# lxd99/TPNet

Measured on AMD Instinct MI355X. Metric: temporal edges/sec (proj-update + pairwise readout), higher is better.
Workload: dtype f32; 1 GPU; C2: Wikipedia-shape d=128 B=1000, L=3, synthetic S(8227,1000,E,span) stream of 2399000 edges, decoder-level unit (2 readouts + update per edge); batch=1000, dim=128, num_layer=3, nodes=9228, parallelism=single GPU

## Files before the change

tpnet_amd/csrc/plan.hip:

```cpp
#include "tpnet_common.h"

#include <cstdlib>
#include <cstring>
#include <rocprim/block/block_radix_sort.hpp>
#include <rocprim/device/device_radix_sort.hpp>
#include <rocprim/device/device_segmented_radix_sort.hpp>
#include <rocprim/iterator/counting_iterator.hpp>
#include <rocprim/iterator/transform_iterator.hpp>

#ifdef TPNET_STAMPS
#define PSTAMP(slot)                                                                          \
    do {                                                                                      \
        if (dbg && blockIdx.x == 0 && threadIdx.x == 0) {                                     \
            dbg[(slot) * 2 + 0] = __builtin_amdgcn_s_memtime();                               \
            dbg[(slot) * 2 + 1] = __builtin_amdgcn_s_memrealtime();                           \
        }                                                                                     \
    } while (0)
#else
#define PSTAMP(slot) do { } while (0)
#endif

namespace tpnet {

static constexpr uint32_t HEAVY_THRESHOLD = 8u;
// ... 900 lines not shown
    if (max_edges < 1) max_edges = 1;
    if (batch < 1) batch = 1;
    return plan_bytes(max_edges, batch) + wplan_extra_bytes(max_edges, batch, N, d, L, 2);
}

int wplan_carve(void* ws, size_t ws_bytes, int64_t Ec, int64_t batch, int64_t N, int d, int L, int K, WPlan* out, float* shared_log,
                bool shard) {
    if (K < 1 || K > WIN_MAX_BATCHES || (!shard && K > wplan_window_batches(batch, d, L))) return TPNET_ERR_BAD_ARG;
    if (Ec > wplan_max_chunk_edges(batch, d, L)) return TPNET_ERR_BAD_ARG;
    int rc = plan_carve(ws, ws_bytes, Ec, batch, &out->base);
    if (rc) return rc;
    const size_t base_bytes = plan_bytes(Ec, batch);
    if (base_bytes + wplan_extra_bytes(Ec, batch, N, d, L, K) - (shared_log ? wplan_log_bytes(Ec, d, L) : 0) > ws_bytes)
        return TPNET_ERR_WORKSPACE;
    char* p = reinterpret_cast<char*>(align_up(reinterpret_cast<size_t>(ws), 256)) + align_up(base_bytes, 256);
    auto take = [&](size_t bytes) -> void* {
        void* r = p;
        p += align_up(bytes, 256);
        return r;
    };
    const size_t nc = 2 * (size_t)Ec;
    const int64_t Ew = (int64_t)K * batch;
    const size_t nw = (size_t)((Ec + batch - 1) / batch);
    out->s_ref = (uint32_t*)take(nc * 4);
    out->s_g = (float*)take(nc * 4);
    out->s_dec = (float*)take(nc * 4);
    out->s_bc = (uint16_t*)take(nc * 2);
    out->wdesc = (WinDesc*)take(nw * sizeof(WinDesc));
    (void)take(256);
    out->e_ref = (uint32_t*)take(3 * (size_t)Ec * 4);
    out->e_g = (float*)take(3 * (size_t)Ec * 4);
    out->log = shared_log ? shared_log : (float*)take(nc * (size_t)L * (size_t)d * 4);
    out->node_lo = (uint32_t*)take((size_t)N * 4);
    out->node_hi = (uint32_t*)take((size_t)N * 4);
    out->inv = (uint32_t*)take(nc * 4);
    out->rhead = (uint32_t*)take(nc * 4);
    out->wmask = (unsigned long long*)take((size_t)N * 8);
    out->wcls = (uint32_t*)take((2 * WIN_MAX_WINDOWS * 8 + WIN_MAX_WINDOWS) * 4);
    out->wzero_bytes = (size_t)(p - reinterpret_cast<char*>(out->wmask));
    out->wtab = take(wplan3_table_bytes(Ec, batch));
    out->wblk = (uint32_t*)take(wplan3_blk_bytes(Ec, batch));
    {
        const size_t db = wplan_dense_bytes(Ec, batch, N, d, L);
        out->dense = db ? take(db) : nullptr;
    }
    out->heavy_thr = wplan_heavy_threshold(K, batch, d);
    out->chains = reinterpret_cast<Chain*>(out->base.light);
    out->chains_sparse = reinterpret_cast<Chain*>(out->base.heavy);
    out->lk_in = reinterpret_cast<uint32_t*>(out->base.keys_in);
    out->lk_out = out->lk_in + nc;
    out->lv_in = out->base.vals_in;
    out->lv_out = out->base.vals_out;
    out->K = K;
    out->Ew = Ew;
    if (p > reinterpret_cast<char*>(ws) + ws_bytes) return TPNET_ERR_WORKSPACE;
    return TPNET_OK;
}

template <typename K>
__global__ void k_make_keys_w(K* __restrict__ keys, uint32_t* __restrict__ vals, const int64_t* __restrict__ src,
                              const int64_t* __restrict__ dst, int64_t Ec, int64_t B, int64_t N, int batch_bits, DescArgs da) {
    if (blockIdx.x >= da.kblocks) {
        for (int64_t b = (int64_t)(blockIdx.x - da.kblocks) * blockDim.x + threadIdx.x; b < da.nb;
             b += (int64_t)(gridDim.x - da.kblocks) * blockDim.x)
            batch_desc(b, da.desc, da.t, Ec, B, da.nb, da.now_time, da.t_prev, da.lambda, da.L);
        return;
    }
    const int64_t nc = 2 * Ec;
    for (int64_t j = (int64_t)blockIdx.x * blockDim.x + threadIdx.x; j < nc; j += (int64_t)da.kblocks * blockDim.x) {
        int64_t b, e;
        int side;
// ... 103 lines not shown
                           const NodeMeta* __restrict__ meta, uint32_t* err) {
    const int64_t nc = 2 * Ec;
    const int KW = p.K;
    const K bmask = ((K)1 << batch_bits) - 1;
    const BatchDesc* __restrict__ desc = p.base.desc;
    for (int64_t jb = (int64_t)bx * blockDim.x; jb < nc; jb += (int64_t)nbx * blockDim.x) {
        const int64_t j = jb + threadIdx.x;
        const bool active = j < nc;
        bool chain_head = false, last_run = false;
        int64_t w = 0;
        if (active) lv[j] = (uint32_t)j;
        Chain ch;
        ch.j0 = 0; ch.cnt = 0; ch.target = 0; ch.prev_ref = WREF_TABLE; ch.g_first = 1.0f; ch.pad0 = 0; ch.pad1 = 0; ch.pad2 = 0;
        if (active) {
            const K key = keys[j];
            const uint32_t val = p.base.vals_out[j];
            const int64_t b = (int64_t)(key & bmask);
            const int64_t node = (int64_t)(key >> batch_bits);
            w = b / KW;
            const double Tb = desc[b].t_last;
            int32_t partner;
            float wgt;
            contribution(p.base, src, dst, t, Ec, B, N, lambda, val, partner, wgt, err);
            p.base.s_partner[j] = partner;
            p.base.s_coef[j] = wgt;
            p.s_bc[j] = (uint16_t)b;
            p.base.s_target[j] = (int32_t)node;

            const bool has_prev = j > 0, has_next = j < nc - 1;
            const K kp = has_prev ? keys[j - 1] : key, kn = has_next ? keys[j + 1] : key;
            const bool run_head = !has_prev || kp != key;
            const bool run_tail = !has_next || kn != key;
            const bool same_node_prev = has_prev && (kp >> batch_bits) == (key >> batch_bits);
            const bool same_node_next = has_next && (kn >> batch_bits) == (key >> batch_bits);
            chain_head = !same_node_prev || (int64_t)(kp & bmask) / KW != w;
            last_run = run_tail && !same_node_next;
            const int64_t h = p.rhead[j];
            const int64_t ri = j - h;
            uint32_t ref;
            float g;
            {
                int64_t cb, ce;
                int cside;
                decode((int64_t)val, B, Ec, cb, cside, ce);
                const int64_t e0b = cb * B;
                const int64_t neb = (Ec - e0b < B) ? (Ec - e0b) : B;
                const uint32_t sym = (uint32_t)(2 * e0b + (cside ? 0 : neb) + (ce - e0b));
                if (!version_before_own_run<K>(p, keys, batch_bits, (int64_t)partner, b, p.inv[sym], desc, meta, lambda, Tb, ref, g))
                    resolve_version(keys, nc, batch_bits, (int64_t)partner, b, desc, meta, lambda, Tb, ref, g, p.node_lo, p.node_hi);
            }
            uint32_t fl = 0;
            if (run_head) fl |= WREF_RUN_HEAD;
            if (run_tail) fl |= WREF_RUN_TAIL;
            if (ri % WIN_BLOCK == 0) fl |= WREF_BLK_HEAD;
            if (ri % WIN_BLOCK == WIN_BLOCK - 1 || run_tail) fl |= WREF_BLK_TAIL;
            if (last_run) fl |= WREF_LAST_RUN;
            p.s_ref[j] = ref | fl;
            p.s_g[j] = g;
            float dec = 1.0f;
            if (run_head && same_node_prev) dec = decay_f32(lambda, Tb - desc[(int64_t)(kp & bmask)].t_last);
            p.s_dec[j] = dec;

            if (chain_head) {
                const K bound = (K)(((uint64_t)node << batch_bits) | (uint64_t)((w + 1) * KW));
                const K node_end = (K)(((uint64_t)(node + 1)) << batch_bits);
                const K stop = ((uint64_t)((w + 1) * KW) > (uint64_t)bmask) ? node_end : bound;
                int64_t lo = j, hi, step = 1;
                for (;;) {
                    const int64_t nx = lo + step;
                    if (nx >= nc) { hi = nc; break; }
                    if (keys[nx] >= stop) { hi = nx; break; }
                    lo = nx;
                    step <<= 1;
                }
                while (hi - lo > 1) {
                    const int64_t mid = (lo + hi) >> 1;
                    if (keys[mid] < stop) lo = mid; else hi = mid;
                }
                ch.j0 = (uint32_t)j;
                ch.cnt = (uint32_t)(hi - j);
                ch.target = (int32_t)node;
                if (same_node_prev) {
                    ch.prev_ref = (uint32_t)(j - 1);
                    ch.g_first = 1.0f;
// ... 160 lines not shown
```

tpnet_amd/csrc/tpnet_common.h:

```cpp
#pragma once
#include <hip/hip_runtime.h>
#include <stdint.h>
#include <stdlib.h>
#include <initializer_list>
#include <new>
#include "../../include/tpnet_hip.h"
#include "tpnet_dev.h"
#include "event_set.hpp"

#ifdef TPNET_DEV
static inline int tpnet_dev_env_int(const char* name, int dflt) { const char* v = getenv(name); return v ? atoi(v) : dflt; }
#define TPNET_DEV_INT(NAME, DFLT) tpnet_dev_env_int("TPNET_DEV_" #NAME, (DFLT))
#define TPNET_DEV_STR(NAME) getenv("TPNET_DEV_" #NAME)
#else
#define TPNET_DEV_INT(NAME, DFLT) (DFLT)
#define TPNET_DEV_STR(NAME) ((const char*)nullptr)
#endif

namespace tpnet {

struct NodeMeta {
    uint32_t ver;
    uint32_t pad0;
    double tref[2];
// ... 197 lines not shown
    return 1 + (dl > 6 ? 6 : (dl < 0 ? 0 : dl));
}

struct WinDesc {
    uint32_t start;
    uint32_t n_heavy;
    uint32_t n_chains;
    uint32_t n_ext;
    uint32_t n_ext1;
    uint32_t n_med;
    uint32_t pad1, pad2;
};

struct Chain {
    uint32_t j0;
    uint32_t cnt;
    int32_t target;
    uint32_t prev_ref;
    float g_first;
    uint32_t pad0, pad1, pad2;
};
static_assert(sizeof(Chain) == 32, "Chain must be 32 bytes");

struct WPlan {
    Plan base;
    uint32_t* s_ref;
    float* s_g;
    float* s_dec;
    uint16_t* s_bc;
    WinDesc* wdesc;
    Chain* chains;
    Chain* chains_sparse;
    uint32_t* lk_in;
    uint32_t* lk_out;
    uint32_t* lv_in;
    uint32_t* lv_out;
    uint32_t* e_ref;
    float* e_g;
    float* log;
    uint32_t* node_lo;
    uint32_t* node_hi;
    uint32_t* inv;
    uint32_t* rhead;
    unsigned long long* wmask;
    uint32_t* wcls;
    void* wtab;
    size_t wzero_bytes;
    uint32_t* wblk;
    void* dense;
    uint32_t heavy_thr;
    int32_t K;
    int64_t Ew;
// ... 63 lines not shown
```

tpnet_amd/csrc/wplan3.hip:

```cpp
#include "wplan_common.hpp"

namespace tpnet {

size_t wplan3_table_bytes(int64_t Ec, int64_t batch) {
    const size_t nb = (size_t)((Ec + batch - 1) / batch);
    return wplan3_h2_bytes(Ec) + 256 + nb * wplan3_seg(batch) * sizeof(HEnt) + 256;
}
size_t wplan3_blk_bytes(int64_t Ec, int64_t batch) {
    const size_t nblk = (size_t)((Ec + batch - 1) / batch) * wplan3_bpb(batch);
    return 2 * nblk * 9 * sizeof(uint32_t) + 256;
}

template <int BS, int IPT>
__global__ __launch_bounds__(BS) void k_wsort(WTmp q, BatchDesc* __restrict__ desc, const int64_t* __restrict__ src_c,
                                              const int64_t* __restrict__ dst_c, const double* __restrict__ t_c, int64_t Ec,
                                              int32_t Bfull, int64_t N, int node_bits, double now_time,
                                              const double* __restrict__ t_prev, double lambda, int L, uint32_t* err, int KW) {
    __shared__ WSortShared<BS, IPT> sh;
    wsort_batch<BS, IPT, false>(sh, q, desc, src_c, dst_c, t_c, Ec, Bfull, N, node_bits, now_time, t_prev, lambda, L, err, KW,
                                (int64_t)blockIdx.x, nullptr);
}


__global__ __launch_bounds__(256) void k_wchains(WPlan p, WTmp q, int64_t Ec, int64_t Bfull, int64_t nb, uint32_t bpb) {
// ... 174 lines not shown
    o.fl = q.bflags[x];
    o.coef = q.bcoef[x];
    o.sb = q.bsb[x - o.ri];
    o.aux = q.rprevb[x - o.ri];
}

__device__ __forceinline__ void side_version(const WPlan& p, const WTmp& q, int64_t Bfull, int64_t w, const CEnt* ce,
                                             const NodeMeta* __restrict__ meta, OwnSide& o) {
    int64_t lb;
    chain_of(p, q, Bfull, ce, w, o.base, o.cnt, lb);
    if (o.sb) {
        o.ver.ref = o.base + o.sb - 1u;
        o.ver.t_src = p.base.desc[o.aux].t_last;
    } else {
        o.ver = version_before_window_m(p, q, Bfull, o.node, w, o.wm, meta);
    }
}

__device__ __forceinline__ void side_store(const WPlan& p, const WTmp& q, int64_t Bfull, int64_t Ec, int64_t e, int sd, int64_t b,
                                           int64_t w, int64_t e0b, double Tb, double Tnow, double lambda,
                                           const NodeMeta* __restrict__ meta, const uint32_t* cabs, int want_edges,
                                           const OwnSide me, const OwnSide other) {
    const uint32_t f = me.base + me.sb + me.ri;
    p.base.s_partner[f] = me.partner;
    p.base.s_coef[f] = me.coef;
    p.base.s_target[f] = (int32_t)me.node;
    p.s_bc[f] = (uint16_t)b;
    VRef pr = other.ver;
    if ((uint32_t)me.partner != other.node)
        pr = version_before_batch(p, q, Bfull, (int64_t)me.partner, b, meta);
    uint32_t out = (me.fl & WT_STRUCT_MASK) | pr.ref;
    float dec = 1.0f;
    if (me.fl & WREF_RUN_HEAD) {
        if (me.fl & WT_CHAIN_HEAD) {
            float g_first = 1.0f;
            if (me.ver.ref & WREF_TABLE) g_first = decay3_f32(lambda, Tb - me.ver.t_src);
            else dec = decay3_f32(lambda, Tb - me.ver.t_src);
            const int c = wchain_class(me.cnt, p.heavy_thr);
            const int64_t blk = b * q.bpb + (me.x - 2 * e0b) / 256;
            uint4* rec = reinterpret_cast<uint4*>(p.chains + (cabs[w * WCLS + c] + q.blkbase[blk * 9 + c] + me.aux));
            rec[0] = make_uint4(f, me.cnt, me.node, me.ver.ref);
            rec[1] = make_uint4(__float_as_uint(g_first), 0u, 0u, 0u);
        } else {
            dec = decay3_f32(lambda, Tb - me.ver.t_src);
        }
    }
    if ((me.fl & WT_WIN_LAST) && (w >= 63 || (me.wm >> (unsigned)(w + 1)) == 0ull)) out |= WREF_LAST_RUN;
    p.s_ref[f] = out;
    p.s_g[f] = decay3_f32(lambda, Tb - pr.t_src);
    p.s_dec[f] = dec;
    if (want_edges) {
        p.e_ref[(int64_t)sd * Ec + e] = me.ver.ref;
        p.e_g[(int64_t)sd * Ec + e] = decay3_f32(lambda, Tnow - me.ver.t_src);
    }
}

__global__ __launch_bounds__(256) void k_wrefs(WPlan p, WTmp q, const int64_t* __restrict__ neg, int64_t Ec, int64_t Bfull,
                                               int64_t nb, int64_t N, double lambda, const NodeMeta* __restrict__ meta,
                                               uint32_t fgrid, int want_edges) {
    const int KW = p.K;
    const BatchDesc* __restrict__ desc = p.base.desc;
    if (blockIdx.x >= fgrid) {
        for (int64_t e = (int64_t)(blockIdx.x - fgrid) * blockDim.x + threadIdx.x; e < Ec;
             e += (int64_t)(gridDim.x - fgrid) * blockDim.x) {
            int64_t node = neg[e];
            if ((uint64_t)node >= (uint64_t)N) node = 0;
            const int64_t b = e / Bfull;
            const VRef r = version_before_batch(p, q, Bfull, node, b, meta);
            p.e_ref[2 * Ec + e] = r.ref;
            p.e_g[2 * Ec + e] = decay3_f32(lambda, desc[b].now - r.t_src);
        }
        return;
    }
// ... 161 lines not shown
```

tpnet_amd/csrc/wplan_common.hpp:

```cpp
#pragma once
#include "tpnet_common.h"
#include "device_common.hpp"

#include <rocprim/block/block_radix_sort.hpp>

namespace tpnet {

static constexpr uint32_t WT_CHAIN_HEAD = 1u;
static constexpr uint32_t WT_WIN_LAST = 2u;
static constexpr uint32_t WT_STRUCT_MASK = WREF_RUN_HEAD | WREF_RUN_TAIL | WREF_BLK_HEAD | WREF_BLK_TAIL;
static constexpr int WCLS = 8;

struct HEnt {
    unsigned long long key;
    uint32_t a, b;
};
static_assert(sizeof(HEnt) == 16, "HEnt must be 16 bytes");
struct CEnt {
    unsigned long long key;
    unsigned long long mask;
    uint32_t xh;
    uint32_t cnt;
    uint32_t pad0, pad1;
};
static_assert(sizeof(CEnt) == 32, "CEnt must be 32 bytes");

#ifdef TPNET_STAMPS
#define WSTAMP(slot)                                                                          \
    do {                                                                                      \
// ... 24 lines not shown
    uint32_t n2;
    uint32_t* blkcnt;
    uint32_t* blkbase;
    uint32_t* boff;
    uint32_t* wtot;
    uint32_t bpb;
    unsigned long long* dbg;
};

static inline uint32_t wplan3_table_entries(size_t nc) { return (uint32_t)(2 * nc + 1021); }
static inline uint32_t wplan3_nc_block(int64_t batch) {
    const int64_t n2 = 2 * batch;
    return n2 <= 512 ? 512u : n2 <= 1024 ? 1024u : n2 <= 2048 ? 2048u : 4096u;
}
static inline uint32_t wplan3_seg(int64_t batch) { return wplan3_nc_block(batch) * 3; }
static inline size_t wplan3_h2_bytes(int64_t Ec) { return (size_t)wplan3_table_entries(2 * (size_t)Ec) * sizeof(CEnt); }
static inline uint32_t wplan3_bpb(int64_t batch) { return (uint32_t)((2 * batch + 255) / 256); }

static WTmp wtmp_of(const WPlan& p, size_t nc) {
    WTmp q;
    q.dbg = p.base.dbg;
    uint32_t* ki = reinterpret_cast<uint32_t*>(p.base.keys_in);
    uint32_t* ko = reinterpret_cast<uint32_t*>(p.base.keys_out);
    uint32_t* hv = reinterpret_cast<uint32_t*>(p.base.heavy);
    q.bkey = ki;
    q.bpart = reinterpret_cast<int32_t*>(ki + nc);
    q.bcoef = reinterpret_cast<float*>(ko);
    q.bval = p.base.vals_out;
    q.binv = p.inv;
    q.bsb = hv;
    q.bri = hv + nc;
    q.rprevb = hv + 2 * nc;
    q.bflags = hv + 3 * nc;
    const uint32_t cap = wplan3_table_entries(nc);
    q.h2 = reinterpret_cast<CEnt*>(p.wtab);
    q.h1 = reinterpret_cast<HEnt*>(reinterpret_cast<char*>(p.wtab) + (wplan3_h2_bytes((int64_t)(nc / 2)) + 255) / 256 * 256);
    q.hcap = cap;
    q.seg = 0;
    q.direct2 = 0;
    q.n2 = 0;
    q.boff = p.rhead;
    q.wtot = p.wcls;
    return q;
}

__device__ __forceinline__ float decay3_f32(double lambda, double dt) {
    const float x = (float)(-lambda * dt);
    return (x == 0.0f) ? 1.0f : expf(x);
}

__device__ __forceinline__ uint32_t hmix(unsigned long long k) {
    k ^= k >> 33;
    k *= 0xff51afd7ed558ccdULL;
    k ^= k >> 33;
    k *= 0xc4ceb9fe1a85ec53ULL;
    k ^= k >> 33;
// ... 293 lines not shown
```

tpnet_amd/csrc/wplan_dense.hip:

```cpp
#include "wplan_dense.hpp"

namespace tpnet {

static constexpr int64_t DENSE_SHARD_MAX_BATCH = 8192;
bool wplan_dense_eligible(int64_t N, int d, int L, int64_t batch) {
    static const int off = TPNET_DEV_INT(NO_PLAN_DENSE, 0);
    if (off || batch < 1 || batch > DENSE_SHARD_MAX_BATCH || N > (int64_t)DENSE_MAX_CHUNKS * 256) return false;
    return (int64_t)N * 12 <= batch * (int64_t)L * d * 4;
}

size_t wplan_dense_bytes(int64_t Ec, int64_t batch, int64_t N, int d, int L) {
    if (!wplan_dense_eligible(N, d, L, batch)) return 0;
    const size_t nb = (size_t)((Ec + batch - 1) / batch);
    const size_t Ns = (size_t)dense_ns(N);
    size_t nw = (nb + 1) / 2 + 1;
    if (nw > (size_t)DENSE_MAX_WINDOWS) nw = DENSE_MAX_WINDOWS;
    const size_t nchunks = (Ns + 255) / 256;
    auto al = [](size_t x) { return (x + 255) / 256 * 256; };
    return al(nb * Ns * 2) + al(nb * Ns * 8) + al(nw * Ns * 4) + al(nw * Ns * 8) + 4 * al(Ns * 4) + al(nchunks * 4) +
           2 * al(nchunks * nw * 8 * 4) + al(nw * 8 * 4) + 256;
}

struct DArgs {
    const int64_t* src;
// ... 15 lines not shown
                                            const double* tl, int64_t x) {
    const BatchDesc* __restrict__ desc = p.base.desc;
    const int KW = p.K;
    const int64_t b = x / (2 * a.Bfull);
    const int64_t e0b = b * a.Bfull;
    const int64_t neb = (a.Ec - e0b < a.Bfull) ? (a.Ec - e0b) : a.Bfull;
    const uint32_t node = q.bkey[x];
    const int32_t partner = q.bpart[x];
    const float coef = q.bcoef[x];
    const uint32_t ri = q.bri[x];
    const uint32_t fl = q.bflags[x] & WT_STRUCT_MASK;
    const uint32_t val = q.bval[x];
    const uint2 mo = D.m[b * D.Ns + node];
    const uint2 mp = D.m[b * D.Ns + (uint32_t)partner];
    const uint2 wsl_own = (fl & WREF_RUN_HEAD) ? D.wsl[(b / KW) * D.Ns + node] : make_uint2(0u, 0u);
    const uint32_t bo = D.base[node] + cbase[node / (uint32_t)DCH];
    const uint32_t bp = D.base[(uint32_t)partner] + cbase[(uint32_t)partner / (uint32_t)DCH];
    const uint4 o0 = reinterpret_cast<const uint4*>(a.meta + node)[0], o1 = reinterpret_cast<const uint4*>(a.meta + node)[1];
    const uint4 p0 = reinterpret_cast<const uint4*>(a.meta + partner)[0], p1 = reinterpret_cast<const uint4*>(a.meta + partner)[1];
    const double Tb = desc[b].t_last, Tnow = desc[b].now;
    const DVRef own = dense_version(desc, tl, mo, bo, o0, o1);
    const DVRef pr = dense_version(desc, tl, mp, bp, p0, p1);
    const uint32_t f = bo + mo.x + ri;
    p.base.s_partner[f] = partner;
    p.base.s_coef[f] = coef;
    p.base.s_target[f] = (int32_t)node;
    p.s_bc[f] = (uint16_t)b;
    uint32_t out = fl | pr.ref;
    float dec = 1.0f;
    if (fl & WREF_RUN_HEAD) {
        const int64_t w = b / KW;
        const uint32_t prevb = mo.y >> 16;
        const bool chain_head = mo.x == 0u || (int64_t)prevb < w * KW;
        if (chain_head) {
            float g_first = 1.0f;
            if (own.ref & WREF_TABLE) g_first = decay3_f32(a.lambda, Tb - own.t_src);
            else dec = decay3_f32(a.lambda, Tb - own.t_src);
            const uint32_t cnt = wsl_own.x;
            const int c = wchain_class(cnt, p.heavy_thr);
            const uint32_t pair = (uint32_t)w * 8u + (uint32_t)c;
            const uint32_t chunk = node / (uint32_t)DCH;
            const uint32_t at = lstart[pair] + D.cpre[(size_t)chunk * (size_t)(a.nw * 8) + pair] + D.crank[w * D.Ns + node];
            uint4* rec = reinterpret_cast<uint4*>(p.chains + at);
            rec[0] = make_uint4(f, cnt, node, own.ref);
            rec[1] = make_uint4(__float_as_uint(g_first), 0u, 0u, 0u);
        } else {
            dec = decay3_f32(a.lambda, Tb - own.t_src);
        }
    }
    if ((fl & WREF_RUN_TAIL) && D.lastb[node] == (uint32_t)b) out |= WREF_LAST_RUN;
    p.s_ref[f] = out;
    p.s_g[f] = decay3_f32(a.lambda, Tb - pr.t_src);
    p.s_dec[f] = dec;
    if (a.nwhich >= 2) {
        const bool side = val >= (uint32_t)neb;
        const int64_t e = e0b + (side ? (int64_t)val - neb : (int64_t)val);
        p.e_ref[(side ? a.Ec : 0) + e] = own.ref;
        p.e_g[(side ? a.Ec : 0) + e] = decay3_f32(a.lambda, Tnow - own.t_src);
    }
}

__device__ __forceinline__ void dense_neg(const WPlan& p, const DView& D, const DArgs& a, const uint32_t* __restrict__ basef,
                                          int64_t e) {
    const BatchDesc* __restrict__ desc = p.base.desc;
    int64_t node = a.neg[e];
    if ((uint64_t)node >= (uint64_t)a.N) node = 0;
    const int64_t b = e / a.Bfull;
    const uint2 m = D.m[b * D.Ns + node];
    const uint32_t bs = basef[node];
    const uint4 m0 = reinterpret_cast<const uint4*>(a.meta + node)[0], m1 = reinterpret_cast<const uint4*>(a.meta + node)[1];
    const DVRef r = dense_version(desc, nullptr, m, bs, m0, m1);
    p.e_ref[2 * a.Ec + e] = r.ref;
    p.e_g[2 * a.Ec + e] = decay3_f32(a.lambda, desc[b].now - r.t_src);
}

__device__ __forceinline__ void dense_neg_c(const WPlan& p, const DView& D, const DArgs& a, const uint32_t* __restrict__ cbase,
// ... 674 lines not shown
```

tpnet_amd/csrc/wstep.hip:

```cpp
#include "readout.hpp"

namespace tpnet {

static constexpr int WB = 256;
#ifndef TPNET_WPIPE_MINW
#define TPNET_WPIPE_MINW 4
#endif
constexpr int wpipe_min_waves(int lpp, int vpl, int l, bool full) {
    return (lpp <= 32 && vpl == 1) ? TPNET_WPIPE_MINW
         : (lpp == 32 && vpl == 2) ? ((full && l <= 3) ? 3 : 2)
         : (lpp == 64 && vpl == 1) ? (full ? 3 : 2)
         : 2;
}

__device__ __forceinline__ float pow_rep(float g, int n) {
    float r = 1.0f;
    for (int z = 0; z < n; ++z) r *= g;
    return r;
}

__device__ __forceinline__ const float* partner_row(const tpnet_state& S, const WPlan& P, int layer, int32_t pv,
                                                    uint32_t ref, float g, float& gp) {
    const int d = S.d, L = S.L;
    if (layer == 1) {
// ... 6 lines not shown
}

__device__ __forceinline__ const float* chain_start(const tpnet_state& S, const WPlan& P, const Chain& c, int layer,
                                                    float& g0) {
    const int d = S.d, L = S.L;
    g0 = pow_rep(c.g_first, layer);
    if (c.prev_ref & WREF_TABLE)
        return S.q + (((int64_t)(c.prev_ref & 1u) * S.N + c.target) * L + (layer - 1)) * (int64_t)d;
    return P.log + ((int64_t)(c.prev_ref & WREF_SLOT_MASK) * L + (layer - 1)) * (int64_t)d;
}

template <int LPP, int VPL, bool FULL>
__device__ __forceinline__ void chain_light(const tpnet_state& S, const WPlan& P, Chain c, bool valid, int layer,
                                            double lambda, int gl, unsigned long long* dbg) {
    (void)dbg;
    STAMP(5);
    constexpr int W = 4, F = VPL * W, U = (F == 4) ? 8 : 4;
    const int d = S.d, L = S.L;
    const int nvec = d / W;
    if (!valid) { c.cnt = 0; c.target = 0; c.j0 = 0; c.prev_ref = WREF_TABLE; c.g_first = 1.0f; }
    float g0;
    const float* qold = chain_start(S, P, c, layer, g0);
    const bool from_table = (c.prev_ref & WREF_TABLE) != 0;
    const int32_t* __restrict__ s_partner = P.base.s_partner;
    const float* __restrict__ s_coef = P.base.s_coef;

    for (int c0 = 0; c0 < (FULL ? 1 : nvec); c0 += LPP * VPL) {
        float acc[F], sblk[F], srun[F];
#pragma unroll
        for (int j = 0; j < VPL; ++j) {
            const int vi = c0 + j * LPP + gl;
            ldv_maybe<W, FULL>(qold, vi, valid && vi < nvec, &acc[j * W]);
        }
#pragma unroll
        for (int x = 0; x < F; ++x) { sblk[x] = 0.0f; srun[x] = 0.0f; }
        bool firstblk = false;
        float cur_dec = 1.0f;
        int32_t nx_pv = 0;
        float nx_w = 0.0f, nx_glog = 1.0f, nx_decr = 1.0f;
        uint32_t nx_ref = 0u;
        auto fetch_meta = [&](uint32_t r0) {
            const uint32_t jm = c.j0 + r0 + (uint32_t)gl;
            const bool mine = r0 + (uint32_t)gl < c.cnt;
            nx_pv = mine ? s_partner[jm] : 0;
            nx_w = mine ? s_coef[jm] : 0.0f;
            nx_ref = mine ? P.s_ref[jm] : 0u;
            nx_glog = mine ? P.s_g[jm] : 1.0f;
            nx_decr = mine ? P.s_dec[jm] : 1.0f;
        };
        fetch_meta(0u);
        for (uint32_t r0 = 0; __any(r0 < c.cnt); r0 += LPP) {
            const int32_t my_pv = nx_pv;
            const float my_w = nx_w;
            const uint32_t my_ref = nx_ref;
            const float my_glog = nx_glog;
            const float my_dec = pow_rep(nx_decr, layer);
            if (__any(r0 + LPP < c.cnt)) fetch_meta(r0 + LPP);
            float my_gp;
            const float* my_row = partner_row(S, P, layer, my_pv, my_ref, my_glog, my_gp);
            const uint32_t n_here = (r0 < c.cnt) ? ((c.cnt - r0 < (uint32_t)LPP) ? c.cnt - r0 : (uint32_t)LPP) : 0u;
            constexpr int US = U / 2;
            float rA[US][F], rB[US][F];
            auto issue = [&](uint32_t k0, float (&r)[US][F]) {
#pragma unroll
                for (int k = 0; k < US; ++k) {
                    const int sl = (int)k0 + k;
                    const bool ok = (uint32_t)sl < n_here;
                    const float* rp = reinterpret_cast<const float*>(__shfl((long long)reinterpret_cast<uintptr_t>(my_row), sl, LPP));
                    if (!ok) rp = S.p0;
#pragma unroll
                    for (int j = 0; j < VPL; ++j) {
// ... 109 lines not shown
    float* r_decp = reinterpret_cast<float*>(lds_u + H::O_DECP);
    uint32_t* task_off = lds_u + H::O_TOFF;
    uint32_t* rlist = lds_u + H::O_RLIST;
    uint32_t* nrun_p = lds_u + H::O_NRUN;
    uint32_t* r_toff = lds_u + H::O_RTOFF;
    uint32_t* r_slot = lds_u + H::O_RSLOT;
    float* r_sum = reinterpret_cast<float*>(lds_u + H::O_RSUM);
    HRec* rec = reinterpret_cast<HRec*>(lds_u + H::O_REC);
    float* lds_part = reinterpret_cast<float*>(lds_u + H::O_PART);
    uint32_t* t_pos = lds_u + H::O_TPOS;
    uint32_t* t_n = lds_u + H::O_TN;

    __syncthreads();
    if (tid < 64) { run_start[tid] = 0xFFFFFFFFu; run_end[tid] = 0u; r_decp[tid] = 1.0f; }
    __syncthreads();
    float* dec_bw = r_sum;
    for (uint32_t p0 = 0; p0 < c.cnt; p0 += 8 * WB) {
        uint32_t ref[8], bcq[8];
        float dec[8];
#pragma unroll
        for (int q = 0; q < 8; ++q) {
            const uint32_t p = p0 + (uint32_t)(q * WB + tid);
            const bool in = p < c.cnt;
            ref[q] = in ? P.s_ref[c.j0 + p] : 0u;
            dec[q] = in ? P.s_dec[c.j0 + p] : 1.0f;
            bcq[q] = in ? (uint32_t)P.s_bc[c.j0 + p] : b0;
        }
#pragma unroll
        for (int q = 0; q < 8; ++q) {
            const uint32_t p = p0 + (uint32_t)(q * WB + tid);
            const uint32_t bw = (bcq[q] - b0) & 63u;
            if (ref[q] & WREF_RUN_HEAD) { run_start[bw] = p; dec_bw[bw] = dec[q]; }
            if (ref[q] & WREF_RUN_TAIL) run_end[bw] = p;
        }
    }
    __syncthreads();
    if (tid < 64) {
        const uint32_t st = run_start[tid];
        const bool has = st != 0xFFFFFFFFu;
        const uint32_t nt = has ? (run_end[tid] - st + WIN_BLOCK) / WIN_BLOCK : 0u;
        uint32_t inc = nt;
#pragma unroll
        for (int o = 1; o < 64; o <<= 1) {
            const uint32_t v = (uint32_t)__shfl_up((int)inc, o, 64);
            if (tid >= o) inc += v;
        }
        task_off[tid] = inc - nt;
        if (tid == 63) task_off[64] = inc;
        const unsigned long long hm = __ballot(has);
// ... 28 lines not shown
            uint32_t lo = 0, hi = 64;
            while (hi - lo > 1) {
                const uint32_t mid = (lo + hi) >> 1;
                if (task_off[mid] <= tt) lo = mid; else hi = mid;
            }
            const uint32_t ps = run_start[lo] + WIN_BLOCK * (tt - task_off[lo]);
            const uint32_t left = run_end[lo] + 1 - ps;
            t_pos[tt - T0] = ps;
            t_n[tt - T0] = left < (uint32_t)WIN_BLOCK ? left : (uint32_t)WIN_BLOCK;
        }
        __syncthreads();
        for (uint32_t x0 = 0; x0 < (Tend - T0) * WIN_BLOCK; x0 += 4 * WB) {
            int32_t pv[4];
            float w[4], glog[4];
            uint32_t ref[4];
            bool in[4];
#pragma unroll
            for (int q = 0; q < 4; ++q) {
                const uint32_t x = x0 + (uint32_t)(q * WB + tid);
                const uint32_t ti = x / WIN_BLOCK, k = x % WIN_BLOCK;
                const bool ok = ti < Tend - T0 && k < t_n[ti < Tend - T0 ? ti : 0];
                in[q] = ok;
                const uint32_t jm = c.j0 + (ok ? t_pos[ti] + k : 0u);
                pv[q] = ok ? P.base.s_partner[jm] : 0;
                w[q] = ok ? P.base.s_coef[jm] : 0.0f;
                ref[q] = ok ? P.s_ref[jm] : 0u;
                glog[q] = ok ? P.s_g[jm] : 1.0f;
            }
#pragma unroll
            for (int q = 0; q < 4; ++q) {
                const uint32_t x = x0 + (uint32_t)(q * WB + tid);
                HRec r;
                bool in_log;
                r.row = partner_row_index(S, layer, pv[q], ref[q], glog[q], r.gp, in_log);
                r.w = in_log ? __uint_as_float(__float_as_uint(w[q]) | 0x80000000u) : w[q];
                if (!in[q]) { r.row = 0xFFFFFFFFu; r.w = 0.0f; r.gp = 0.0f; }
                if (x < (Tend - T0) * WIN_BLOCK) rec[x] = r;
            }
        }
        __syncthreads();
        for (uint32_t tb = T0; tb < Tend; tb += G * HT) {
            float sb[HT][4];
            bool act[HT];
#pragma unroll
            for (int h = 0; h < HT; ++h) {
                const uint32_t tt = tb + (uint32_t)(h * G + g);
                act[h] = tt < Tend;
                const HRec* rr = rec + (size_t)((act[h] ? tt : T0) - T0) * WIN_BLOCK;
                float r[WIN_BLOCK][4], w[WIN_BLOCK], gp[WIN_BLOCK];
                bool ok[WIN_BLOCK];
// ... 149 lines not shown
    uint32_t* b_slot = lds_u + M::O_BSLOT;
    uint32_t* own = lds_u + M::O_OWN;
    uint32_t* misc = lds_u + M::O_MISC;
    float* bsum = reinterpret_cast<float*>(lds_u + M::O_SUM);

    float g0;
    const float* qold = chain_start(S, P, c, layer, g0);
    const bool from_table = (c.prev_ref & WREF_TABLE) != 0;
    float acc[F], srun[F];
#pragma unroll
    for (int j = 0; j < VPL; ++j) ldv<W>(g == 0 ? qold : S.p0, j * LPP + gl, &acc[j * W]);
#pragma unroll
    for (int x = 0; x < F; ++x) srun[x] = 0.0f;
    bool firstblk = false;
    float cur_dec = 1.0f;

    for (uint32_t s0 = 0; s0 < c.cnt;) {
        __syncthreads();
        const uint32_t left = c.cnt - s0 < (uint32_t)SEGP ? c.cnt - s0 : (uint32_t)SEGP;
        const uint32_t pg = (left + GPB - 1) / GPB < 2u ? 2u : (left + GPB - 1) / GPB;
        const uint32_t pos = s0 + (uint32_t)tid;
        const bool in = tid < SEGP && pos < c.cnt;
        const uint32_t jm = c.j0 + (in ? pos : 0u);
        const int32_t pv = in ? P.base.s_partner[jm] : 0;
        const float wgt = in ? P.base.s_coef[jm] : 0.0f;
        const uint32_t ref = in ? P.s_ref[jm] : 0u;
        const float glog = in ? P.s_g[jm] : 1.0f;
        const float decr = in ? P.s_dec[jm] : 1.0f;
        if (tid <= GPB) own[tid] = SEGP;
        const bool head = in && (ref & WREF_BLK_HEAD) != 0;
        const unsigned long long hm = __ballot(head);
        const int lane = tid & 63, wave = tid >> 6;
        if (lane == 0 && wave < 4) misc[2 + wave] = (uint32_t)__popcll(hm);
        __syncthreads();
        uint32_t blk = (uint32_t)__popcll(hm & ((2ull << lane) - 1ull)) - 1u;
        for (int wv = 0; wv < wave && wv < 4; ++wv) blk += misc[2 + wv];
        const bool keep = in && blk < (uint32_t)BCAP;
        if (tid < SEGP) {
            float gp;
            const float* row = partner_row(S, P, layer, pv, ref, glog, gp);
            p_row[tid] = row;
            p_w[tid] = wgt;
            p_gp[tid] = gp;
            p_fl[tid] = keep ? ref : 0u;
            p_dec[tid] = pow_rep(decr, layer);
            p_blk[tid] = blk;
        }
        if (keep && head) {
            atomicMin(&own[(uint32_t)tid / pg], (uint32_t)tid);
            b_fl[blk] = (ref & WREF_RUN_HEAD) ? 1u : 0u;
            b_dec[blk] = (pos == 0u && from_table) ? g0 : pow_rep(decr, layer);
// ... 270 lines not shown
    const int64_t n_small = (int64_t)wd.n_chains - (int64_t)n_hub;
    for (int64_t base = (int64_t)rb * GPB; base < n_small; base += (int64_t)nblk * GPB) {
        const int64_t idx = base + g;
        const bool valid = idx < n_small;
        const Chain c = small[valid ? idx : 0];
        chain_light<LPP, VPL, FULL>(S, P, c, valid, layer, lambda, gl, dbg);
    }
    BEND();
}

static constexpr int WBS = 256;
__global__ __launch_bounds__(WB) void k_wwriteback(tpnet_state S, WPlan P, int64_t nc, uint32_t bid) {
    const int per = S.L * S.d;
    NodeMeta* meta = reinterpret_cast<NodeMeta*>(S.meta);
    __shared__ uint32_t n_list;
    __shared__ uint32_t l_pos[WBS];
    __shared__ int32_t l_node[WBS];
    __shared__ int32_t l_copy[WBS];
    for (int64_t j0 = (int64_t)blockIdx.x * WBS; j0 < nc; j0 += (int64_t)gridDim.x * WBS) {
        __syncthreads();
        if (threadIdx.x == 0) n_list = 0;
        __syncthreads();
        const int64_t j = j0 + threadIdx.x;
        if (threadIdx.x < WBS && j < nc && (P.s_ref[j] & WREF_LAST_RUN)) {
            const int32_t u = P.base.s_target[j];
            const int c = (int)(meta[u].ver & 1u);
            const uint32_t k = atomicAdd(&n_list, 1u);
            l_pos[k] = (uint32_t)j;
            l_node[k] = u;
            l_copy[k] = c;
        }
        __syncthreads();
        const uint32_t n = n_list;
        if ((per & 3) == 0) {
            const uint32_t pv = (uint32_t)per / 4;
            const uint32_t tot = n * pv;
            for (uint32_t x0 = threadIdx.x; x0 < tot; x0 += 4 * WB) {
                const uint32_t xa = x0, xb = x0 + WB, xc = x0 + 2 * WB, xd = x0 + 3 * WB;
                const uint32_t ka = xa / pv, kb = (xb < tot ? xb : xa) / pv, kc = (xc < tot ? xc : xa) / pv, kd = (xd < tot ? xd : xa) / pv;
                const uint32_t oa = xa - ka * pv, ob = (xb < tot ? xb : xa) - kb * pv, oc = (xc < tot ? xc : xa) - kc * pv,
                               od = (xd < tot ? xd : xa) - kd * pv;
                const float4 va = reinterpret_cast<const float4*>(P.log + (int64_t)l_pos[ka] * per)[oa];
                const float4 vb = reinterpret_cast<const float4*>(P.log + (int64_t)l_pos[kb] * per)[ob];
                const float4 vc = reinterpret_cast<const float4*>(P.log + (int64_t)l_pos[kc] * per)[oc];
                const float4 vd = reinterpret_cast<const float4*>(P.log + (int64_t)l_pos[kd] * per)[od];
                reinterpret_cast<float4*>(S.q + ((int64_t)(l_copy[ka] ^ 1) * S.N + l_node[ka]) * (int64_t)per)[oa] = va;
                if (xb < tot) reinterpret_cast<float4*>(S.q + ((int64_t)(l_copy[kb] ^ 1) * S.N + l_node[kb]) * (int64_t)per)[ob] = vb;
                if (xc < tot) reinterpret_cast<float4*>(S.q + ((int64_t)(l_copy[kc] ^ 1) * S.N + l_node[kc]) * (int64_t)per)[oc] = vc;
                if (xd < tot) reinterpret_cast<float4*>(S.q + ((int64_t)(l_copy[kd] ^ 1) * S.N + l_node[kd]) * (int64_t)per)[od] = vd;
            }
        } else {
            for (uint32_t x = threadIdx.x; x < n * (uint32_t)per; x += WB) {
                const uint32_t k = x / (uint32_t)per, o = x - k * (uint32_t)per;
                S.q[((int64_t)(l_copy[k] ^ 1) * S.N + l_node[k]) * (int64_t)per + o] = P.log[(int64_t)l_pos[k] * per + o];
            }
        }
        if (threadIdx.x < n) {
            const uint32_t k = threadIdx.x;
            publish_meta(meta + l_node[k], l_copy[k] ^ 1, P.base.desc[P.s_bc[l_pos[k]]].t_last, bid);
        }
    }
}

int launch_wwriteback(const tpnet_state& st, const WPlan& p, int64_t Ec, int64_t, uint32_t launch_id, hipStream_t s, int64_t) {
    const int64_t nc = 2 * Ec;
    int64_t grid = (nc + WBS - 1) / WBS;
    if (grid > 16384) grid = 16384;
    if (grid < 1) grid = 1;
    hipLaunchKernelGGL(k_wwriteback, dim3((unsigned)grid), dim3(WB), 0, s, st, p, nc, launch_id);
    TPNET_HIP_TRY(hipGetLastError());
    return TPNET_OK;
}

int launch_wstep(const tpnet_state& st, const StreamArgs& a, const WPlan& p, int64_t j, int64_t Ec, int64_t batch,
                 double lambda, uint32_t flags, hipStream_t s) {
    if ((reinterpret_cast<uintptr_t>(a.out_pos) | reinterpret_cast<uintptr_t>(a.out_neg)) & 15) return TPNET_ERR_BAD_ARG;
    if (st.d % 4 != 0) return TPNET_ERR_BAD_ARG;
    const int L = st.L;
    const int64_t nw = (Ec + p.Ew - 1) / p.Ew;
    static const int hb_env = TPNET_DEV_INT(WIN_HB, 0);
    static const int stamp_layer = TPNET_DEV_INT(STAMP_LAYER, 0);
    static const int geo_env = TPNET_DEV_INT(WIN_GEOM, 0);
// ... 95 lines not shown
```

Before: 346.4 million edges/s.

## Pack per-slot plan metadata into a 32-byte record (AoS) for vectorized access

Replaces seven separate per-slot arrays (partner, coef, ref, g, dec, target, bc) with one 32-byte WRec struct written as two uint4 stores and read as uint4 loads. The plan builders, the dense and wplan3 paths, the step kernels and the writeback all switch to the packed record, and the scratch buffers are moved to make room. The aim is fewer memory transactions and better coalescing per slot. In exchange, readers that need only one or two fields now fetch a full 16-byte half, which wastes bandwidth in the writeback and ref-only loops. Unused fields are also loaded unconditionally.

```diff
diff --git a/tpnet_amd/csrc/plan.hip b/tpnet_amd/csrc/plan.hip
--- a/tpnet_amd/csrc/plan.hip
+++ b/tpnet_amd/csrc/plan.hip
@@ -1,4 +1,4 @@
-#include "tpnet_common.h"
+#include "wplan_common.hpp"
 
 #include <cstdlib>
 #include <cstring>
@@ -946,10 +946,8 @@
     const size_t nc = 2 * (size_t)Ec;
     const int64_t Ew = (int64_t)K * batch;
     const size_t nw = (size_t)((Ec + batch - 1) / batch);
-    out->s_ref = (uint32_t*)take(nc * 4);
-    out->s_g = (float*)take(nc * 4);
-    out->s_dec = (float*)take(nc * 4);
-    out->s_bc = (uint16_t*)take(nc * 2);
+    out->wscr = (uint32_t*)take(3 * align_up(nc * 4, 256));
+    (void)take(nc * 2);
     out->wdesc = (WinDesc*)take(nw * sizeof(WinDesc));
     (void)take(256);
     out->e_ref = (uint32_t*)take(3 * (size_t)Ec * 4);
@@ -970,7 +968,9 @@
     }
     out->heavy_thr = wplan_heavy_threshold(K, batch, d);
     out->chains = reinterpret_cast<Chain*>(out->base.light);
-    out->chains_sparse = reinterpret_cast<Chain*>(out->base.heavy);
+    static_assert(sizeof(WRec) == sizeof(Item), "WPlan::rec takes the place of Plan::heavy");
+    out->rec = reinterpret_cast<WRec*>(out->base.heavy);
+    out->chains_sparse = reinterpret_cast<Chain*>(out->wtab);
     out->lk_in = reinterpret_cast<uint32_t*>(out->base.keys_in);
     out->lk_out = out->lk_in + nc;
     out->lv_in = out->base.vals_in;
@@ -1120,10 +1120,6 @@
             int32_t partner;
             float wgt;
             contribution(p.base, src, dst, t, Ec, B, N, lambda, val, partner, wgt, err);
-            p.base.s_partner[j] = partner;
-            p.base.s_coef[j] = wgt;
-            p.s_bc[j] = (uint16_t)b;
-            p.base.s_target[j] = (int32_t)node;
 
             const bool has_prev = j > 0, has_next = j < nc - 1;
             const K kp = has_prev ? keys[j - 1] : key, kn = has_next ? keys[j + 1] : key;
@@ -1153,11 +1149,9 @@
             if (ri % WIN_BLOCK == 0) fl |= WREF_BLK_HEAD;
             if (ri % WIN_BLOCK == WIN_BLOCK - 1 || run_tail) fl |= WREF_BLK_TAIL;
             if (last_run) fl |= WREF_LAST_RUN;
-            p.s_ref[j] = ref | fl;
-            p.s_g[j] = g;
             float dec = 1.0f;
             if (run_head && same_node_prev) dec = decay_f32(lambda, Tb - desc[(int64_t)(kp & bmask)].t_last);
-            p.s_dec[j] = dec;
+            wrec_store(p.rec, (size_t)j, partner, wgt, ref | fl, g, dec, (int32_t)node, (uint32_t)b);
 
             if (chain_head) {
                 const K bound = (K)(((uint64_t)node << batch_bits) | (uint64_t)((w + 1) * KW));
diff --git a/tpnet_amd/csrc/tpnet_common.h b/tpnet_amd/csrc/tpnet_common.h
--- a/tpnet_amd/csrc/tpnet_common.h
+++ b/tpnet_amd/csrc/tpnet_common.h
@@ -243,12 +243,22 @@
 };
 static_assert(sizeof(Chain) == 32, "Chain must be 32 bytes");
 
+struct WRec {
+    int32_t partner;
+    float coef;
+    uint32_t ref;
+    float g;
+    float dec;
+    int32_t target;
+    uint32_t bc;
+    uint32_t spare;
+};
+static_assert(sizeof(WRec) == 32, "WRec must be 32 bytes");
+
 struct WPlan {
     Plan base;
-    uint32_t* s_ref;
-    float* s_g;
-    float* s_dec;
-    uint16_t* s_bc;
+    WRec* rec;
+    uint32_t* wscr;
     WinDesc* wdesc;
     Chain* chains;
     Chain* chains_sparse;
diff --git a/tpnet_amd/csrc/wplan3.hip b/tpnet_amd/csrc/wplan3.hip
--- a/tpnet_amd/csrc/wplan3.hip
+++ b/tpnet_amd/csrc/wplan3.hip
@@ -220,10 +220,6 @@
                                            const NodeMeta* __restrict__ meta, const uint32_t* cabs, int want_edges,
                                            const OwnSide me, const OwnSide other) {
     const uint32_t f = me.base + me.sb + me.ri;
-    p.base.s_partner[f] = me.partner;
-    p.base.s_coef[f] = me.coef;
-    p.base.s_target[f] = (int32_t)me.node;
-    p.s_bc[f] = (uint16_t)b;
     VRef pr = other.ver;
     if ((uint32_t)me.partner != other.node)
         pr = version_before_batch(p, q, Bfull, (int64_t)me.partner, b, meta);
@@ -244,9 +240,7 @@
         }
     }
     if ((me.fl & WT_WIN_LAST) && (w >= 63 || (me.wm >> (unsigned)(w + 1)) == 0ull)) out |= WREF_LAST_RUN;
-    p.s_ref[f] = out;
-    p.s_g[f] = decay3_f32(lambda, Tb - pr.t_src);
-    p.s_dec[f] = dec;
+    wrec_store(p.rec, f, me.partner, me.coef, out, decay3_f32(lambda, Tb - pr.t_src), dec, (int32_t)me.node, (uint32_t)b);
     if (want_edges) {
         p.e_ref[(int64_t)sd * Ec + e] = me.ver.ref;
         p.e_g[(int64_t)sd * Ec + e] = decay3_f32(lambda, Tnow - me.ver.t_src);
diff --git a/tpnet_amd/csrc/wplan_common.hpp b/tpnet_amd/csrc/wplan_common.hpp
--- a/tpnet_amd/csrc/wplan_common.hpp
+++ b/tpnet_amd/csrc/wplan_common.hpp
@@ -5,6 +5,32 @@
 #include <rocprim/block/block_radix_sort.hpp>
 
 namespace tpnet {
+
+__device__ __forceinline__ void wrec_store(WRec* __restrict__ rec, size_t f, int32_t partner, float coef, uint32_t ref, float g,
+                                           float dec, int32_t target, uint32_t bc) {
+    uint4* r = reinterpret_cast<uint4*>(rec + f);
+    r[0] = make_uint4((uint32_t)partner, __float_as_uint(coef), ref, __float_as_uint(g));
+    r[1] = make_uint4(__float_as_uint(dec), (uint32_t)target, bc, 0u);
+}
+struct WRecWalk {
+    int32_t partner;
+    float coef;
+    uint32_t ref;
+    float g;
+};
+struct WRecEnds {
+    float dec;
+    int32_t target;
+    uint32_t bc;
+};
+__device__ __forceinline__ WRecWalk wrec_load_walk(const WRec* __restrict__ rec, size_t f) {
+    const uint4 v = reinterpret_cast<const uint4*>(rec + f)[0];
+    return {(int32_t)v.x, __uint_as_float(v.y), v.z, __uint_as_float(v.w)};
+}
+__device__ __forceinline__ WRecEnds wrec_load_ends(const WRec* __restrict__ rec, size_t f) {
+    const uint4 v = reinterpret_cast<const uint4*>(rec + f)[1];
+    return {__uint_as_float(v.x), (int32_t)v.y, v.z};
+}
 
 static constexpr uint32_t WT_CHAIN_HEAD = 1u;
 static constexpr uint32_t WT_WIN_LAST = 2u;
@@ -75,16 +101,15 @@
     q.dbg = p.base.dbg;
     uint32_t* ki = reinterpret_cast<uint32_t*>(p.base.keys_in);
     uint32_t* ko = reinterpret_cast<uint32_t*>(p.base.keys_out);
-    uint32_t* hv = reinterpret_cast<uint32_t*>(p.base.heavy);
     q.bkey = ki;
     q.bpart = reinterpret_cast<int32_t*>(ki + nc);
     q.bcoef = reinterpret_cast<float*>(ko);
     q.bval = p.base.vals_out;
     q.binv = p.inv;
-    q.bsb = hv;
-    q.bri = hv + nc;
-    q.rprevb = hv + 2 * nc;
-    q.bflags = hv + 3 * nc;
+    q.bsb = p.wscr;
+    q.bri = p.wscr + nc;
+    q.rprevb = p.wscr + 2 * nc;
+    q.bflags = p.base.vals_in;
     const uint32_t cap = wplan3_table_entries(nc);
     q.h2 = reinterpret_cast<CEnt*>(p.wtab);
     q.h1 = reinterpret_cast<HEnt*>(reinterpret_cast<char*>(p.wtab) + (wplan3_h2_bytes((int64_t)(nc / 2)) + 255) / 256 * 256);
diff --git a/tpnet_amd/csrc/wplan_dense.hip b/tpnet_amd/csrc/wplan_dense.hip
--- a/tpnet_amd/csrc/wplan_dense.hip
+++ b/tpnet_amd/csrc/wplan_dense.hip
@@ -61,10 +61,6 @@
     const DVRef own = dense_version(desc, tl, mo, bo, o0, o1);
     const DVRef pr = dense_version(desc, tl, mp, bp, p0, p1);
     const uint32_t f = bo + mo.x + ri;
-    p.base.s_partner[f] = partner;
-    p.base.s_coef[f] = coef;
-    p.base.s_target[f] = (int32_t)node;
-    p.s_bc[f] = (uint16_t)b;
     uint32_t out = fl | pr.ref;
     float dec = 1.0f;
     if (fl & WREF_RUN_HEAD) {
@@ -88,9 +84,7 @@
         }
     }
     if ((fl & WREF_RUN_TAIL) && D.lastb[node] == (uint32_t)b) out |= WREF_LAST_RUN;
-    p.s_ref[f] = out;
-    p.s_g[f] = decay3_f32(a.lambda, Tb - pr.t_src);
-    p.s_dec[f] = dec;
+    wrec_store(p.rec, f, partner, coef, out, decay3_f32(a.lambda, Tb - pr.t_src), dec, (int32_t)node, (uint32_t)b);
     if (a.nwhich >= 2) {
         const bool side = val >= (uint32_t)neb;
         const int64_t e = e0b + (side ? (int64_t)val - neb : (int64_t)val);
diff --git a/tpnet_amd/csrc/wstep.hip b/tpnet_amd/csrc/wstep.hip
--- a/tpnet_amd/csrc/wstep.hip
+++ b/tpnet_amd/csrc/wstep.hip
@@ -1,4 +1,5 @@
 #include "readout.hpp"
+#include "wplan_common.hpp"
 
 namespace tpnet {
 
@@ -52,8 +53,7 @@
     float g0;
     const float* qold = chain_start(S, P, c, layer, g0);
     const bool from_table = (c.prev_ref & WREF_TABLE) != 0;
-    const int32_t* __restrict__ s_partner = P.base.s_partner;
-    const float* __restrict__ s_coef = P.base.s_coef;
+    const WRec* __restrict__ rec = P.rec;
 
     for (int c0 = 0; c0 < (FULL ? 1 : nvec); c0 += LPP * VPL) {
         float acc[F], sblk[F], srun[F];
@@ -72,11 +72,13 @@
         auto fetch_meta = [&](uint32_t r0) {
             const uint32_t jm = c.j0 + r0 + (uint32_t)gl;
             const bool mine = r0 + (uint32_t)gl < c.cnt;
-            nx_pv = mine ? s_partner[jm] : 0;
-            nx_w = mine ? s_coef[jm] : 0.0f;
-            nx_ref = mine ? P.s_ref[jm] : 0u;
-            nx_glog = mine ? P.s_g[jm] : 1.0f;
-            nx_decr = mine ? P.s_dec[jm] : 1.0f;
+            const WRecWalk rw = wrec_load_walk(rec, mine ? jm : c.j0);
+            const WRecEnds re = wrec_load_ends(rec, mine ? jm : c.j0);
+            nx_pv = mine ? rw.partner : 0;
+            nx_w = mine ? rw.coef : 0.0f;
+            nx_ref = mine ? rw.ref : 0u;
+            nx_glog = mine ? rw.g : 1.0f;
+            nx_decr = mine ? re.dec : 1.0f;
         };
         fetch_meta(0u);
         for (uint32_t r0 = 0; __any(r0 < c.cnt); r0 += LPP) {
@@ -232,9 +234,11 @@
         for (int q = 0; q < 8; ++q) {
             const uint32_t p = p0 + (uint32_t)(q * WB + tid);
             const bool in = p < c.cnt;
-            ref[q] = in ? P.s_ref[c.j0 + p] : 0u;
-            dec[q] = in ? P.s_dec[c.j0 + p] : 1.0f;
-            bcq[q] = in ? (uint32_t)P.s_bc[c.j0 + p] : b0;
+            const WRecWalk rw = wrec_load_walk(P.rec, c.j0 + (in ? p : 0u));
+            const WRecEnds re = wrec_load_ends(P.rec, c.j0 + (in ? p : 0u));
+            ref[q] = in ? rw.ref : 0u;
+            dec[q] = in ? re.dec : 1.0f;
+            bcq[q] = in ? re.bc : b0;
         }
 #pragma unroll
         for (int q = 0; q < 8; ++q) {
@@ -309,10 +313,11 @@
                 const bool ok = ti < Tend - T0 && k < t_n[ti < Tend - T0 ? ti : 0];
                 in[q] = ok;
                 const uint32_t jm = c.j0 + (ok ? t_pos[ti] + k : 0u);
-                pv[q] = ok ? P.base.s_partner[jm] : 0;
-                w[q] = ok ? P.base.s_coef[jm] : 0.0f;
-                ref[q] = ok ? P.s_ref[jm] : 0u;
-                glog[q] = ok ? P.s_g[jm] : 1.0f;
+                const WRecWalk rw = wrec_load_walk(P.rec, jm);
+                pv[q] = ok ? rw.partner : 0;
+                w[q] = ok ? rw.coef : 0.0f;
+                ref[q] = ok ? rw.ref : 0u;
+                glog[q] = ok ? rw.g : 1.0f;
             }
 #pragma unroll
             for (int q = 0; q < 4; ++q) {
@@ -508,11 +513,13 @@
         const uint32_t pos = s0 + (uint32_t)tid;
         const bool in = tid < SEGP && pos < c.cnt;
         const uint32_t jm = c.j0 + (in ? pos : 0u);
-        const int32_t pv = in ? P.base.s_partner[jm] : 0;
-        const float wgt = in ? P.base.s_coef[jm] : 0.0f;
-        const uint32_t ref = in ? P.s_ref[jm] : 0u;
-        const float glog = in ? P.s_g[jm] : 1.0f;
-        const float decr = in ? P.s_dec[jm] : 1.0f;
+        const WRecWalk rw = wrec_load_walk(P.rec, jm);
+        const WRecEnds re = wrec_load_ends(P.rec, jm);
+        const int32_t pv = in ? rw.partner : 0;
+        const float wgt = in ? rw.coef : 0.0f;
+        const uint32_t ref = in ? rw.ref : 0u;
+        const float glog = in ? rw.g : 1.0f;
+        const float decr = in ? re.dec : 1.0f;
         if (tid <= GPB) own[tid] = SEGP;
         const bool head = in && (ref & WREF_BLK_HEAD) != 0;
         const unsigned long long hm = __ballot(head);
@@ -829,8 +836,8 @@
         if (threadIdx.x == 0) n_list = 0;
         __syncthreads();
         const int64_t j = j0 + threadIdx.x;
-        if (threadIdx.x < WBS && j < nc && (P.s_ref[j] & WREF_LAST_RUN)) {
-            const int32_t u = P.base.s_target[j];
+        if (threadIdx.x < WBS && j < nc && (wrec_load_walk(P.rec, (size_t)j).ref & WREF_LAST_RUN)) {
+            const int32_t u = wrec_load_ends(P.rec, (size_t)j).target;
             const int c = (int)(meta[u].ver & 1u);
             const uint32_t k = atomicAdd(&n_list, 1u);
             l_pos[k] = (uint32_t)j;
@@ -864,7 +871,7 @@
         }
         if (threadIdx.x < n) {
             const uint32_t k = threadIdx.x;
-            publish_meta(meta + l_node[k], l_copy[k] ^ 1, P.base.desc[P.s_bc[l_pos[k]]].t_last, bid);
+            publish_meta(meta + l_node[k], l_copy[k] ^ 1, P.base.desc[wrec_load_ends(P.rec, l_pos[k]).bc].t_last, bid);
         }
     }
 }
```

Measured after the change: 365.3 million edges/s, median of 6. 1.05x the previous value.
